# nvpro-samples/vk_raytrace

Measured on AMD Instinct MI355X. Metric: Msamples/s on Sponza 1920x1080; per-pixel L2 vs ref at equal spp, higher is better.
Workload: dtype f32; 1 GPU; C3 sponza-like (synthetic Crytek-Sponza stand-in, 262267 tris target) 1920x1080 589spp depth8 Disney + HDR env; triangles=269004, materials=23, textures=43, width=1920, height=1080, spp=589, max_depth=8, bsdf=disney, env=2048x1024 procedural HDR, parallelism=image tiles 32x32 over 1 GPU(s), scene replicated

## Files before the change

include/pt_fpmath.h:

```cpp
#ifndef PT_FPMATH_H
#define PT_FPMATH_H

#include <math.h>
#include <stdint.h>
#include <string.h>

#if defined(__HIPCC__)
#define PT_FP __host__ __device__ __forceinline__
#else
#define PT_FP static inline
#endif

PT_FP float ptf_from_bits(uint32_t u)
{
  float f;
  memcpy(&f, &u, 4);
  return f;
}
PT_FP uint32_t ptf_bits(float f)
{
  uint32_t u;
  memcpy(&u, &f, 4);
  return u;
}
// ... 49 lines not shown
  if(ptf_abs(x) < 2.44140625e-4f)
    return x;
  float r;
  int   q;
  ptf_sincos_reduce(x, &r, &q);
  float v = (q & 1) ? ptf_cos_kernel(r) : ptf_sin_kernel(r);
  return (q & 2) ? -v : v;
}
PT_FP float pt_cos(float x)
{
  float r;
  int   q;
  ptf_sincos_reduce(x, &r, &q);
  float v = (q & 1) ? ptf_sin_kernel(r) : ptf_cos_kernel(r);
  return ((q + 1) & 2) ? -v : v;
}
PT_FP float pt_tan(float x)
{
  if(ptf_abs(x) < 2.44140625e-4f)
    return x;
  float r;
  int   q;
  ptf_sincos_reduce(x, &r, &q);
  float s = ptf_sin_kernel(r), c = ptf_cos_kernel(r);
  return (q & 1) ? -c / s : s / c;
}

PT_FP float ptf_asin_poly(float x, float z)
{
  float p = ptf_fma(3.3921066672e-02f, z, 1.7005795613e-02f);
// ... 262 lines not shown
```

include/pt_types.h:

```cpp
#ifndef PT_TYPES_H
#define PT_TYPES_H

#include <stdint.h>

#ifdef __cplusplus
extern "C" {
#endif

#define PT_TILE 32

enum pt_DebugMode {
  PT_DEBUG_NONE = 0,
  PT_DEBUG_BASECOLOR = 1,
  PT_DEBUG_NORMAL = 2,
  PT_DEBUG_METALLIC = 3,
  PT_DEBUG_EMISSIVE = 4,
  PT_DEBUG_ALPHA = 5,
  PT_DEBUG_ROUGHNESS = 6,
  PT_DEBUG_TEXCOORD = 7,
  PT_DEBUG_TANGENT = 8,
  PT_DEBUG_RADIANCE = 9,
  PT_DEBUG_WEIGHT = 10,
  PT_DEBUG_RAYDIR = 11,
  PT_DEBUG_HEATMAP = 12
// ... 121 lines not shown
typedef struct pt_PrimMesh {
  uint32_t vertexOffset;
  uint32_t vertexCount;
  uint32_t firstIndex;
  uint32_t indexCount;
  int32_t  materialIndex;
} pt_PrimMesh;

typedef struct pt_Node {
  float   worldMatrix[16];
  int32_t primMesh;
} pt_Node;

enum { PT_VARIANT_RAYQUERY = 0, PT_VARIANT_RTX = 1 };
enum { PT_ACCEL_FLAT = 0, PT_ACCEL_TWO_LEVEL = 1 };
enum { PT_FN_SIN = 0, PT_FN_COS, PT_FN_TAN, PT_FN_ASIN, PT_FN_ACOS, PT_FN_ATAN2, PT_FN_EXP, PT_FN_LOG, PT_FN_POW };
enum { PT_FILTER_NEAREST = 0, PT_FILTER_LINEAR = 1 };
enum { PT_WRAP_REPEAT = 0, PT_WRAP_MIRRORED_REPEAT = 1, PT_WRAP_CLAMP_TO_EDGE = 2 };

typedef struct pt_TextureDesc {
  const uint8_t* rgba8;
  int32_t        width;
  int32_t        height;
  int32_t        magFilter;
  int32_t        minFilter;
  int32_t        wrapS;
  int32_t        wrapT;
} pt_TextureDesc;

typedef struct pt_SceneDesc {
  const pt_VertexAttributes*  vertices;
// ... 108 lines not shown
```

vk_raytrace_amd/capi.py:

```python
import ctypes as C
import os

import numpy as np

from . import host_device as hd

PT_VARIANT_RAYQUERY, PT_VARIANT_RTX = 0, 1
PT_ACCEL_FLAT, PT_ACCEL_TWO_LEVEL = 0, 1
PT_RAYS_CLOSEST, PT_RAYS_OCCLUDED, PT_RAYS_NEAREST, PT_RAYS_CANDIDATES = 0, 1, 2, 3
PT_RAY_HIT, PT_RAY_INVALID = 1, 2
PT_RAYS_DEVICE = 1
PT_RAYS_MAX_HITS = 16
PT_QUERY_CHUNK = 1 << 20
PT_DISPLAY_RING = 8
PT_FN = {"sin": 0, "cos": 1, "tan": 2, "asin": 3, "acos": 4, "atan2": 5, "exp": 6, "log": 7, "pow": 8}
PT_OK, PT_ERR_INVALID, PT_ERR_NO_DEVICE, PT_ERR_HIP, PT_ERR_STATE, PT_ERR_OOM, PT_ERR_UNAVAILABLE = 0, -1, -2, -3, -4, -5, -6

LIB_PATH = os.environ.get("PT_LIB") or os.path.join(os.path.dirname(os.path.abspath(__file__)), "libptmi.so")

_P = C.c_void_p
API = [
    ("pt_create", C.c_int, [C.c_int, C.POINTER(_P)]),
    ("pt_destroy", C.c_int, [_P]),
    ("pt_renderer_name", C.c_char_p, []),
    ("pt_last_error", C.c_char_p, [_P]),
    ("pt_set_scene", C.c_int, [_P, C.POINTER(hd.SceneDesc)]),
    ("pt_build_accel", C.c_int, [_P]),
    ("pt_set_accel_mode", C.c_int, [_P, C.c_int]),
    ("pt_update_instances", C.c_int, [_P, _P, C.c_uint32]),
    ("pt_set_camera", C.c_int, [_P, C.POINTER(hd.SceneCamera)]),
# ... 128 lines not shown
```

vk_raytrace_amd/csrc/pt_bsdf.h:

```cpp
#pragma once
#include "pt_surface.h"

PT_DEV float schlick_weight(float u)
{
  float m  = clampf(1.0f - u, 0.0f, 1.0f);
  float m2 = m * m;
  return m2 * m2 * m;
}
PT_DEV float fresnel_dielectric(float cosI, float eta)
{
  float sinT2 = eta * eta * (1.0f - cosI * cosI);
  if(sinT2 > 1.0f)
    return 1.0f;
  float cosT = sqrtf(fmax2(1.0f - sinT2, 0.0f));
  float rs   = (eta * cosT - cosI) / (eta * cosT + cosI);
  float rp   = (eta * cosI - cosT) / (eta * cosI + cosT);
  return 0.5f * (rs * rs + rp * rp);
}
PT_DEV float gtr1(float NdotH, float a)
{
  if(a >= 1.0f)
    return PT_1_OVER_PI;
  float a2 = a * a;
  float t  = 1.0f + (a2 - 1.0f) * NdotH * NdotH;
// ... 13 lines not shown
  return 1.0f / (PT_PI * ax * ay * c * c);
}
PT_DEV float smith_ggx(float NdotV, float alphaG)
{
  float a = alphaG * alphaG;
  float b = NdotV * NdotV;
  return 1.0f / (NdotV + sqrtf(a + b - a * b));
}
PT_DEV float smith_ggx_aniso(float NdotV, float VdotX, float VdotY, float ax, float ay)
{
  float a = VdotX * ax;
  float b = VdotY * ay;
  float c = NdotV;
  return 1.0f / (NdotV + sqrtf(a * a + b * b + c * c));
}
PT_DEV f3 sample_cosine_hemisphere(float r1, float r2)
{
  float r   = sqrtf(r1);
  float phi = PT_TWO_PI * r2;
  f3    d;
  d.x = r * pt_cos(phi);
  d.y = r * pt_sin(phi);
  d.z = sqrtf(fmax2(0.0f, 1.0f - d.x * d.x - d.y * d.y));
  return d;
}
PT_DEV f3 sample_uniform_hemisphere(float r1, float r2)
{
  float r   = sqrtf(fmax2(0.0f, 1.0f - r1 * r1));
  float phi = PT_TWO_PI * r2;
  return f3{r * pt_cos(phi), r * pt_sin(phi), r1};
}
PT_DEV float power_heuristic(float a, float b)
{
  float t = a * a;
  return t / (b * b + t);
}
PT_DEV f3 sample_gtr1(float rgh, float r1)
{
  float a        = fmax2(0.001f, rgh);
  float a2       = a * a;
  float phi      = r1 * PT_TWO_PI;
  float cosTheta = sqrtf((1.0f - pt_pow(a2, 1.0f - r1)) / (1.0f - a2));
  float sinTheta = clampf(sqrtf(1.0f - (cosTheta * cosTheta)), 0.0f, 1.0f);
  return f3{sinTheta * pt_cos(phi), sinTheta * pt_sin(phi), cosTheta};
}
PT_DEV f3 sample_gtr2_aniso(float ax, float ay, float r1, float r2)
{
  float phi      = r1 * PT_TWO_PI;
  float sinPhi   = ay * pt_sin(phi);
  float cosPhi   = ax * pt_cos(phi);
  float tanTheta = sqrtf(r2 / (1 - r2));
  return f3{tanTheta * cosPhi, tanTheta * sinPhi, 1.0f};
}
PT_DEV f3 sample_gtr2(float rgh, float r1, float r2)
{
  float a        = fmax2(0.001f, rgh);
  float phi      = r1 * PT_TWO_PI;
  float cosTheta = sqrtf((1.0f - r2) / (1.0f + (a * a - 1.0f) * r2));
  float sinTheta = clampf(sqrtf(1.0f - (cosTheta * cosTheta)), 0.0f, 1.0f);
  return f3{sinTheta * pt_cos(phi), sinTheta * pt_sin(phi), cosTheta};
}

PT_DEV f3 disney_reflection(const Surface& s, float eta, f3 V, f3 N, f3 L, f3 H, float& pdf)
{
  if(dot3(N, L) < 0.0f)
    return splat3(0.0f);
  float F = fresnel_dielectric(dot3(V, H), eta);
  float D = gtr2(dot3(N, H), s.roughness);
  pdf     = D * dot3(N, H) * F / (4.0f * dot3(V, H));
  float G = smith_ggx(fabsf(dot3(N, L)), s.roughness) * smith_ggx(dot3(N, V), s.roughness);
  return s.albedo * F * D * G;
}
PT_DEV f3 disney_refraction(const Surface& s, float eta, f3 V, f3 N, f3 L, f3 H, float& pdf)
{
  float F     = fresnel_dielectric(fabsf(dot3(V, H)), eta);
// ... 43 lines not shown
{
  pdf      = (1.0f / PT_TWO_PI);
  float FL = schlick_weight(fabsf(dot3(N, L)));
  float FV = schlick_weight(dot3(N, V));
  float Fd = (1.0f - 0.5f * FL) * (1.0f - 0.5f * FV);
  return sqrt3(s.albedo) * s.subsurface * (1.0f / PT_PI) * Fd * (1.0f - s.metallic) * (1.0f - s.transmission);
}
PT_DEV f3 disney_spec_tint(const Surface& s)
{
  f3    Cdlin = s.albedo;
  float Cdlum = 0.3f * Cdlin.x + 0.6f * Cdlin.y + 0.1f * Cdlin.z;
  f3    Ctint = Cdlum > 0.0f ? Cdlin / Cdlum : splat3(1.0f);
  return lerp(lerp(splat3(1.0f), Ctint, s.specularTint) * (s.specular * 0.08f), Cdlin, s.metallic);
}

PT_DEV f3 disney_sample(const Surface& s, f3 V, f3 N, f3& L, float& pdf, uint32_t& seed)
{
  pdf  = 0.0f;
  f3 f = splat3(0.0f);

  float r1 = rng_next(seed);
  float r2 = rng_next(seed);

  float diffuseRatio = 0.5f * (1.0f - s.metallic);
  float transWeight  = (1.0f - s.metallic) * s.transmission;
  f3    Cspec0       = disney_spec_tint(s);
  f3    Csheen       = s.sheenTint;

  if(rng_next(seed) < transWeight)
  {
    f3 H = sample_gtr2(s.roughness, r1, r2);
    H    = s.tangent * H.x + s.bitangent * H.y + N * H.z;

    f3    R   = mirror(-V, H);
    float eta = s.eta;
    float F   = fresnel_dielectric(fabsf(dot3(R, H)), eta);
    if(s.thinwalled)
    {
      if(dot3(s.ffnormal, s.normal) < 0.0f)
        F = 0;
      eta = 1.001f;
    }
    if(rng_next(seed) < F)
    {
      L = unit(R);
      f = disney_reflection(s, eta, V, N, L, H, pdf);
    }
    else
    {
      L = unit(bend(-V, H, eta));
      f = disney_refraction(s, eta, V, N, L, H, pdf);
    }
    f *= transWeight;
    pdf *= transWeight;
  }
  else
  {
    if(rng_next(seed) < diffuseRatio)
    {
      if(rng_next(seed) < s.subsurface)
      {
        L = sample_uniform_hemisphere(r1, r2);
        L = s.tangent * L.x + s.bitangent * L.y - N * L.z;
        f = disney_subsurface(s, V, N, L, pdf);
        pdf *= s.subsurface * diffuseRatio;
      }
      else
      {
        L    = sample_cosine_hemisphere(r1, r2);
        L    = s.tangent * L.x + s.bitangent * L.y + N * L.z;
        f3 H = unit(L + V);
        f    = disney_diffuse(s, Csheen, V, N, L, H, pdf);
        pdf *= (1.0f - s.subsurface) * diffuseRatio;
      }
    }
    else
    {
      float primarySpecRatio = 1.0f / (1.0f + s.clearcoat);
      if(rng_next(seed) < primarySpecRatio)
      {
        f3 H = sample_gtr2_aniso(s.ax, s.ay, r1, r2);
        H    = s.tangent * H.x + s.bitangent * H.y + N * H.z;
        L    = unit(mirror(-V, H));
        f    = disney_specular(s, Cspec0, V, N, L, H, pdf);
        pdf *= primarySpecRatio * (1.0f - diffuseRatio);
      }
      else
      {
        f3 H = sample_gtr1(s.clearcoatRoughness, r1);
        H    = s.tangent * H.x + s.bitangent * H.y + N * H.z;
        L    = unit(mirror(-V, H));
        f    = disney_clearcoat(s, V, N, L, H, pdf);
        pdf *= (1.0f - primarySpecRatio) * (1.0f - diffuseRatio);
      }
    }
    f *= (1.0f - transWeight);
    pdf *= (1.0f - transWeight);
  }
  return f;
}

PT_DEV f3 disney_eval(const Surface& s, f3 V, f3 N, f3 L, float& pdf)
{
  f3 H;
  if(dot3(N, L) < 0.0f)
    H = unit(L * (1.0f / s.eta) + V);
  else
    H = unit(L + V);
  if(dot3(N, H) < 0.0f)
// ... 59 lines not shown
  return clampf(v, 0.0f, 1.0f);
}
PT_DEV float gltf_d_ggx(float NdotH, float alphaRoughness)
{
  float a2 = alphaRoughness * alphaRoughness;
  float f  = (NdotH * NdotH) * (a2 - 1.0f) + 1.0f;
  return a2 / (PT_PI * f * f);
}
PT_DEV float gltf_d_ggx_aniso(float NdotH, float TdotH, float BdotH, float at, float ab)
{
  float a2 = at * ab;
  f3    f  = f3{ab * TdotH, at * BdotH, a2 * NdotH};
  float w2 = a2 / dot3(f, f);
  return a2 * w2 * w2 / PT_PI;
}
PT_DEV f3 gltf_ggx_halfvector(float alpha, float r1, float r2)
{
  float phi      = r1 * 2.0f * PT_PI;
  float cosTheta = sqrtf((1.0f - r2) / (1.0f + (alpha * alpha - 1.0f) * r2));
  float sinTheta = clampf(sqrtf(1.0f - (cosTheta * cosTheta)), 0.0f, 1.0f);
  return f3{sinTheta * pt_cos(phi), sinTheta * pt_sin(phi), cosTheta};
}
PT_DEV f3 gltf_diffuse(const Surface& s, f3 V, f3 N, f3 L, float& pdf)
{
  pdf         = 0;
  float NdotV = dot3(N, V);
  float NdotL = dot3(N, L);
  if(NdotL < 0.0f || NdotV < 0.0f)
    return splat3(0.0f);
  NdotL = clampf(NdotL, 0.001f, 1.0f);
  pdf   = NdotL * PT_1_OVER_PI;
  return (s.albedo / PT_PI) * (1.0f - s.metallic);
}
PT_DEV f3 gltf_specular(const Surface& s, f3 f0, f3 f90, f3 V, f3 N, f3 L, f3 H, float& pdf)
{
  pdf         = 0;
// ... 91 lines not shown
  return lerp(brdf, bsdf, transWeight);
}

PT_DEV f3 gltf_sample(const Surface& s, f3 V, f3 N, f3& L, float& pdf, uint32_t& seed)
{
  pdf     = 0.0f;
  f3 brdf = splat3(0.0f);

  float probability   = rng_next(seed);
  float diffuseRatio  = 0.5f * (1.0f - s.metallic);
  float specularRatio = 1.0f - diffuseRatio;
  float transWeight   = (1.0f - s.metallic) * s.transmission;
  float r1            = rng_next(seed);
  float r2            = rng_next(seed);

  if(rng_next(seed) < transWeight)
  {
    float eta   = s.eta;
    float n2    = s.ior;
    float R0    = (1.0f - n2) / (1.0f + n2);
    f3    H     = gltf_ggx_halfvector(s.roughness, r1, r2);
    H           = s.tangent * H.x + s.bitangent * H.y + N * H.z;
    float VdotH = dot3(V, H);
    float F     = gltf_fresnel(R0 * R0, 1.0f, VdotH);
    float disc  = 1.0f - eta * eta * (1.0f - VdotH * VdotH);
    if(s.thinwalled)
    {
      if(dot3(s.ffnormal, s.normal) < 0.0f)
      {
        F    = 0;
        disc = 0;
      }
      eta = 1.00f;
    }
    if(disc < 0.0f || rng_next(seed) < F)
    {
// ... 3 lines not shown
    {
      L = unit(bend(-V, H, eta));
      if(isnan(L.x) || isnan(L.y) || isnan(L.z))
        L = -V;
    }
    pdf  = fabsf(dot3(N, L));
    brdf = s.albedo;
  }
  else
  {
    f3 f0, f90;
    gltf_f0_f90(s, f0, f90);
    f3 T = s.tangent, B = s.bitangent;
    if(probability < diffuseRatio)
    {
      L    = sample_cosine_hemisphere(r1, r2);
      L    = T * L.x + B * L.y + N * L.z;
      brdf = gltf_diffuse(s, V, N, L, pdf);
      pdf *= (1.0f - s.subsurface) * diffuseRatio;
    }
    else
    {
      float primarySpecRatio = 1.0f / (1.0f + s.clearcoat);
      float roughness        = (rng_next(seed) < primarySpecRatio) ? s.roughness : s.clearcoatRoughness;
      f3    H                = gltf_ggx_halfvector(roughness, r1, r2);
      H                      = T * H.x + B * H.y + N * H.z;
      L                      = mirror(-V, H);
      if(rng_next(seed) < primarySpecRatio)
      {
        brdf = gltf_specular(s, f0, f90, V, N, L, H, pdf);
        pdf *= primarySpecRatio * specularRatio;
      }
      else
      {
        brdf = gltf_clearcoat(s, V, N, L, H, pdf);
        pdf *= (1.0f - primarySpecRatio) * specularRatio;
      }
    }
    brdf *= (1.0f - transWeight);
    pdf *= (1.0f - transWeight);
// ... 4 lines not shown
```

vk_raytrace_amd/csrc/pt_capi.hip:

```cpp
#include <algorithm>
#include <atomic>
#include <cstdlib>
#include <cstring>
#include "pt_context.h"
#include "pt_scene_records.h"

static std::string g_createError;

int dev_alloc(pt_context* c, DevBuf& b, size_t bytes)
{
  if(b.p && b.bytes >= bytes && b.bytes <= bytes * 2 + 4096)
    return PT_OK;
  dev_free(b);
  if(bytes == 0)
    bytes = 16;
  HIP_TRY(c, hipMalloc(&b.p, bytes));
  b.bytes = bytes;
  return PT_OK;
}
bool dev_alloc_quiet(DevBuf& b, size_t bytes)
{
  if(b.p && b.bytes >= bytes && b.bytes <= bytes * 2 + 4096)
    return true;
  dev_free(b);
// ... 427 lines not shown
}

int pt_set_env(pt_context* c, const float* rgba, int w, int h, float* out_integral, float* out_average)
{
  CTX_CHECK(c);
  if(!rgba || w <= 0 || h <= 0)
    return c->fail(PT_ERR_INVALID, "pt_set_env: bad image");
  HIP_TRY(c, hipSetDevice(c->device));
  HIP_TRY(c, sync_all(c));
  std::vector<pt_EnvAccel> accel(size_t(w) * h);
  float                    integral = 1.f, average = 1.f;
  if(pt_build_env_accel(rgba, w, h, accel.data(), &integral, &average) != PT_OK)
    return c->fail(PT_ERR_INVALID, "pt_build_env_accel failed");
  int rc;
  if((rc = upload(c, c->dEnv, rgba, sizeof(float) * 4 * size_t(w) * h)) != PT_OK) return rc;
  if((rc = upload(c, c->dEnvAccel, accel.data(), sizeof(pt_EnvAccel) * accel.size())) != PT_OK) return rc;
  c->scene.envW = w;
  c->scene.envH = h;
  c->haveEnv    = true;
  refresh_scene_ptrs(c);
  if(out_integral) *out_integral = integral;
  if(out_average) *out_average = average;
  return PT_OK;
}

int pt_set_variant(pt_context* c, int variant)
{
  CTX_CHECK(c);
  if(variant != PT_VARIANT_RAYQUERY && variant != PT_VARIANT_RTX)
    return c->fail(PT_ERR_INVALID, "pt_set_variant: %d", variant);
  int rc = flush_pending(c);
// ... 766 lines not shown
```

vk_raytrace_amd/csrc/pt_debug.hip:

```cpp
#include <algorithm>
#include "pt_context.h"
#include "pt_probe.h"

extern "C" {

__global__ void __launch_bounds__(256) k_calib_valu(int iters, float* out)
{
  float a0 = threadIdx.x, a1 = a0 + 1.f, a2 = a0 + 2.f, a3 = a0 + 3.f, a4 = a0 + 4.f, a5 = a0 + 5.f, a6 = a0 + 6.f, a7 = a0 + 7.f;
  const float m = 0.999f, c = 0.001f;
  for(int i = 0; i < iters; ++i)
  {
    asm volatile("v_fmac_f32 %0, %8, %9\n v_fmac_f32 %1, %8, %9\n v_fmac_f32 %2, %8, %9\n v_fmac_f32 %3, %8, %9\n"
                 "v_fmac_f32 %4, %8, %9\n v_fmac_f32 %5, %8, %9\n v_fmac_f32 %6, %8, %9\n v_fmac_f32 %7, %8, %9\n"
                 : "+v"(a0), "+v"(a1), "+v"(a2), "+v"(a3), "+v"(a4), "+v"(a5), "+v"(a6), "+v"(a7)
                 : "v"(m), "v"(c));
  }
  float s = ((a0 + a1) + (a2 + a3)) + ((a4 + a5) + (a6 + a7));
  if(s == 12345.678f)
    out[0] = s;
}
__global__ void __launch_bounds__(256) k_calib_copy(const float4* __restrict__ src, float4* __restrict__ dst, size_t n)
{
  for(size_t i = size_t(blockIdx.x) * blockDim.x + threadIdx.x; i < n; i += size_t(gridDim.x) * blockDim.x)
    dst[i] = src[i];
// ... 63 lines not shown
{
  uint64_t i = uint64_t(blockIdx.x) * blockDim.x + threadIdx.x;
  if(i >= n)
    return;
  float x = a[i], y = b ? b[i] : 0.0f, r;
  switch(fn)
  {
    case PT_FN_SIN: r = pt_sin(x); break;
    case PT_FN_COS: r = pt_cos(x); break;
    case PT_FN_TAN: r = pt_tan(x); break;
    case PT_FN_ASIN: r = pt_asin(x); break;
    case PT_FN_ACOS: r = pt_acos(x); break;
    case PT_FN_ATAN2: r = pt_atan2(x, y); break;
    case PT_FN_EXP: r = pt_exp(x); break;
    case PT_FN_LOG: r = pt_log(x); break;
    default: r = pt_pow(x, y); break;
  }
  out[i] = r;
}
int pt_fpmath_eval(pt_context* c, int fn, uint64_t n, const float* a, const float* b, float* out)
{
  CTX_CHECK(c);
  if(fn < PT_FN_SIN || fn > PT_FN_POW || !a || !out || ((fn == PT_FN_ATAN2 || fn == PT_FN_POW) && !b))
    return c->fail(PT_ERR_INVALID, "pt_fpmath_eval: bad arguments");
  if(n == 0)
    return PT_OK;
  HIP_TRY(c, hipSetDevice(c->device));
  float *dA = nullptr, *dB = nullptr, *dO = nullptr;
  int    rc = PT_OK;
  auto   done = [&](int r) {
    (void)hipFree(dA); (void)hipFree(dB); (void)hipFree(dO);
    return r;
  };
  if(hipMalloc(&dA, n * 4) != hipSuccess || hipMalloc(&dO, n * 4) != hipSuccess || (b && hipMalloc(&dB, n * 4) != hipSuccess))
    return done(c->fail(PT_ERR_OOM, "pt_fpmath_eval: out of device memory"));
  if(hipMemcpy(dA, a, n * 4, hipMemcpyHostToDevice) != hipSuccess || (b && hipMemcpy(dB, b, n * 4, hipMemcpyHostToDevice) != hipSuccess))
    return done(c->fail(PT_ERR_HIP, "pt_fpmath_eval: upload failed"));
  k_fpmath<<<dim3((unsigned)((n + 255) / 256)), dim3(256), 0, c->stream>>>(fn, n, dA, dB, dO);
  if(hipStreamSynchronize(c->stream) != hipSuccess || hipMemcpy(out, dO, n * 4, hipMemcpyDeviceToHost) != hipSuccess)
    return done(c->fail(PT_ERR_HIP, "pt_fpmath_eval: kernel failed"));
  return done(rc);
}

}

template <class Launch>
static int run_rows(pt_context* c, const char* who, uint32_t n, const float* in, int in_stride, float* out, int out_stride, Launch&& launch)
{
  float *dIn = nullptr, *dOut = nullptr;
  auto   done = [&](int r) {
    (void)hipFree(dIn); (void)hipFree(dOut);
    return r;
  };
  const size_t inBytes = size_t(n) * in_stride * 4, outBytes = size_t(n) * out_stride * 4;
// ... 170 lines not shown
```

vk_raytrace_amd/csrc/pt_device.h:

```cpp
#pragma once
#include "../../include/pt_types.h"
#include "pt_math.h"
#include <cstring>

struct TriRec {
  float4 p0w;
  float4 e1n;
  float4 e2p;
};
#define TRI_OPAQUE 1u
#define TRI_NOCULL 2u
#define TRI_FLIP 4u
#define TRI_INDEX_MASK 0x1fffffffu

struct BvhNode {
  float4 a;
  float4 b;
  float4 c;
  uint4  d;
};
#define BVH_LEAF 0x80000000u
#define BVH_ALPHA 0x40000000u
#define BVH_SLOT_MASK 0x3fffffffu
#define BVH_NONE 0xffffffffu
// ... 138 lines not shown
         eq(m.attenuationColor[2], one) && eq(m.thicknessFactor, zero) && eq(m.attenuationDistance, big) && eq(m.clearcoatFactor, zero) &&
         eq(m.clearcoatRoughness, zero) && m.clearcoatTexture == -1 && m.clearcoatRoughnessTexture == -1 && m.sheen == 0u;
}
inline void mat_line_pack(const pt_GltfShadeMaterial& m, const TexRec rec[4], uint4 out[PT_MAT_LINE_QUADS])
{
  auto bits = [](float f) { uint32_t u; std::memcpy(&u, &f, 4); return u; };
  const int      ids[4] = {m.normalTexture, m.emissiveTexture, m.pbrMetallicRoughnessTexture, m.pbrBaseColorTexture};
  const uint32_t flags  = (ids[0] > -1 ? MAT_HAS_NORMAL : 0u) | (ids[1] > -1 ? MAT_HAS_EMISSIVE : 0u) | (ids[2] > -1 ? MAT_HAS_MR : 0u) | (ids[3] > -1 ? MAT_HAS_BASE : 0u) |
                         (mat_is_simple(m) ? MAT_SIMPLE : 0u);
  out[0] = uint4{bits(m.pbrBaseColorFactor[0]), bits(m.pbrBaseColorFactor[1]), bits(m.pbrBaseColorFactor[2]), bits(m.pbrBaseColorFactor[3])};
  out[1] = uint4{bits(m.emissiveFactor[0]), bits(m.emissiveFactor[1]), bits(m.emissiveFactor[2]), bits(m.normalTextureScale)};
  out[2] = uint4{bits(m.pbrRoughnessFactor), bits(m.pbrMetallicFactor), bits(m.ior), flags};
  for(int k = 0; k < 4; ++k)
    out[3 + k] = tex_desc_pack(rec[k]);
  out[7] = uint4{0u, 0u, 0u, 0u};
}

#define PT_SHADE_REC_QUADS 8
struct DeviceScene {
  const float4*               vertices;
  const uint32_t*             indices;
  const InstanceRec*          instances;
  const pt_GltfShadeMaterial* materials;
  const pt_Light*             lights;
  const TexRec*               texRecs;
  const uint4*                matLines;
  const uint32_t*             texels;
  const BvhNode*              bvh;
  const WideNode*             wide;
  const CompactNode*          cnodes;
  const float4*               shadeTris;
  const TriRec*               tris;
  const AlphaRec*             alphaRecs;
  const AlphaMat*             alphaMats;
  const uint32_t*             alphaMaps;
  const float4*               env;
  const pt_EnvAccel*          envAccel;
  int32_t                     envW, envH;
  uint32_t                    numTris;
  uint32_t                    numInstances;
  pt_SceneCamera              camera;
  pt_SunAndSky                sunsky;
  float                       boundsMin[3];
  float                       boundsInvExt[3];
  const WideNode*             tlas;
  const CompactNode*          ctlas;
  const TlasLeaf*             tlasLeaves;
  const uint32_t*             instTriBase;
  const uint32_t*             instBlock;
  uint32_t                    twoLevel;
  uint32_t                    allOpaque;
};

#define PT_STATE_PLAIN 0
#define PT_STATE_NT 1
#ifndef PT_STATE_POLICY
#define PT_STATE_POLICY PT_STATE_NT
#endif
template <int POL>
struct StateArrayT {
  float4* p;
  PT_DEV float4& operator[](size_t i) const { return p[i]; }
  PT_DEV operator float4*() const { return p; }
};
#if defined(__HIP_DEVICE_COMPILE__)
typedef float pt_nt_f4 __attribute__((ext_vector_type(4)));
struct StateF1RefNt {
// ... 63 lines not shown
```

vk_raytrace_amd/csrc/pt_probe.h:

```cpp
#pragma once
#include "pt_shade.h"
#include "pt_cnode.h"

enum {
  PROBE_EVAL_DISNEY = 0, PROBE_EVAL_GLTF, PROBE_SAMPLE_DISNEY, PROBE_SAMPLE_GLTF, PROBE_SUN_AND_SKY, PROBE_SPHERICAL_UV, PROBE_FRAME, PROBE_RANGE_ATTENUATION,
  PROBE_SPOT_ATTENUATION, PROBE_MIRROR, PROBE_BEND, PROBE_LERP, PROBE_SMOOTH, PROBE_ENV_SAMPLE, PROBE_CROSS, PROBE_UNIT, PROBE_MAT4_VEC4, PROBE_VEC4_MAT4,
  PROBE_XFORM_POINT, PROBE_XFORM_ROWVEC, PROBE_XFORM_DIR, PROBE_BASIS_MUL, PROBE_COUNT
};
enum { PROBE_BSDF_IN = 40, PROBE_ENV_TEXELS = 8, PROBE_SKY_WORDS = int(sizeof(pt_SunAndSky) / 4) };

__host__ __device__ inline void probe_row_words(int fn, int& in, int& out)
{
  switch(fn)
  {
    case PROBE_EVAL_DISNEY: case PROBE_EVAL_GLTF: in = PROBE_BSDF_IN; out = 4; break;
    case PROBE_SAMPLE_DISNEY: case PROBE_SAMPLE_GLTF: in = PROBE_BSDF_IN; out = 8; break;
    case PROBE_SUN_AND_SKY: in = PROBE_SKY_WORDS + 3; out = 3; break;
    case PROBE_SPHERICAL_UV: in = 3; out = 2; break;
    case PROBE_FRAME: in = 3; out = 6; break;
    case PROBE_RANGE_ATTENUATION: in = 2; out = 1; break;
    case PROBE_SPOT_ATTENUATION: in = 8; out = 1; break;
    case PROBE_MIRROR: in = 6; out = 3; break;
    case PROBE_BEND: case PROBE_LERP: in = 7; out = 3; break;
    case PROBE_SMOOTH: in = 3; out = 1; break;
    case PROBE_ENV_SAMPLE: in = 8 + 4 * PROBE_ENV_TEXELS; out = 4; break;
    case PROBE_CROSS: in = 6; out = 3; break;
    case PROBE_UNIT: in = 3; out = 3; break;
    case PROBE_MAT4_VEC4: in = 20; out = 4; break;
    case PROBE_XFORM_POINT: case PROBE_XFORM_ROWVEC: case PROBE_XFORM_DIR: in = 15; out = 3; break;
    case PROBE_BASIS_MUL: in = 12; out = 3; break;
    default: in = 0; out = 0; break;
  }
}

PT_DEV f3 probe_f3(const float* p) { return f3{p[0], p[1], p[2]}; }
PT_DEV void probe_put(float* o, f3 v) { o[0] = v.x; o[1] = v.y; o[2] = v.z; }

PT_DEV void probe_surface(Surface& s, const float* r)
{
  const float* m = r;
// ... 53 lines not shown
    case PROBE_FRAME:
    {
      f3 T, B;
      make_frame(probe_f3(in), T, B);
      probe_put(out, T);
      probe_put(out + 3, B);
      break;
    }
    case PROBE_RANGE_ATTENUATION: out[0] = range_attenuation(in[0], in[1]); break;
    case PROBE_SPOT_ATTENUATION: out[0] = spot_attenuation(probe_f3(in), probe_f3(in + 3), in[6], in[7]); break;
    case PROBE_MIRROR: probe_put(out, mirror(probe_f3(in), probe_f3(in + 3))); break;
    case PROBE_BEND: probe_put(out, bend(probe_f3(in), probe_f3(in + 3), in[6])); break;
    case PROBE_LERP: probe_put(out, lerp(probe_f3(in), probe_f3(in + 3), in[6])); break;
    case PROBE_SMOOTH: out[0] = smooth(in[0], in[1], in[2]); break;
    case PROBE_ENV_SAMPLE:
    {
      const int w = int(in[3]), h = int(in[4]);
      if(w < 1 || h < 1 || w * h > PROBE_ENV_TEXELS)
        break;
      pt_EnvAccel acc[PROBE_ENV_TEXELS];
      float4      texels[PROBE_ENV_TEXELS];
      for(int k = 0; k < PROBE_ENV_TEXELS; ++k)
      {
        acc[k].alias = __float_as_uint(in[8 + 4 * k]); acc[k].q = in[9 + 4 * k]; acc[k].pdf = in[10 + 4 * k]; acc[k].aliasPdf = in[11 + 4 * k];
        texels[k] = make_float4(1.0f, 1.0f, 1.0f, 1.0f);
      }
      DeviceScene S;
      memset(&S, 0, sizeof(S));
      S.env = texels; S.envAccel = acc; S.envW = w; S.envH = h;
      f3    toLight = splat3(0.0f);
      float pdf     = 0.0f;
      (void)env_importance_sample(S, probe_f3(in), toLight, pdf);
      probe_put(out, toLight);
      out[3] = pdf;
      break;
    }
    case PROBE_CROSS: probe_put(out, cross3(probe_f3(in), probe_f3(in + 3))); break;
    case PROBE_UNIT: probe_put(out, unit(probe_f3(in))); break;
    case PROBE_MAT4_VEC4:
    {
      const f4 r = mat4_mul(in, f4{in[16], in[17], in[18], in[19]});
      out[0] = r.x; out[1] = r.y; out[2] = r.z; out[3] = r.w;
      break;
    }
// ... 341 lines not shown
```

vk_raytrace_amd/csrc/pt_shade.h:

```cpp
#pragma once
#include "pt_bsdf.h"
#include "pt_internal.h"
#include "pt_sky.h"
#include "pt_settle.h"

enum { SHADE_DONE = 0, SHADE_TO_SHADOW = 1, SHADE_TO_NEXT = 2 };
enum { EV_MISS = 1u, EV_HIT = 2u, EV_NEE = 4u };

PT_DEV bool slot_pixel(const FrameParams& fp, const uint32_t* slotTile, uint32_t slot, int& px, int& py)
{
  uint32_t gt = slotTile[slot >> 10];
  uint32_t in = slot & 1023u, blk = in >> 6, lane = in & 63u;
  px          = int(gt % uint32_t(fp.tilesX)) * PT_TILE + int(blk & 3u) * 8 + int(lane & 7u);
  py          = int(gt / uint32_t(fp.tilesX)) * PT_TILE + int(blk >> 2) * 8 + int(lane >> 3);
  return px < fp.width && py < fp.height;
}

PT_DEV f4 mat4_mul(const float* m, f4 v)
{
  f4 c0 = f4{m[0], m[1], m[2], m[3]}, c1 = f4{m[4], m[5], m[6], m[7]}, c2 = f4{m[8], m[9], m[10], m[11]}, c3 = f4{m[12], m[13], m[14], m[15]};
  return ((c0 * v.x + c1 * v.y) + c2 * v.z) + c3 * v.w;
}

PT_DEV f2 spherical_uv(f3 v)
// ... 41 lines not shown
  f2 center = f2{float(px), float(py)} + jitter;
  f2 inUV   = f2{center.x / float(st.size[0]), center.y / float(st.size[1])};
  f2 d      = inUV * 2.0f - f2{1.0f, 1.0f};

  const pt_SceneCamera& cam = S.camera;
  f4 origin    = mat4_mul(cam.viewInverse, f4{0, 0, 0, 1});
  f4 target    = mat4_mul(cam.projInverse, f4{d.x, d.y, 1, 1});
  f3 tn        = unit(xyz(target));
  f4 direction = mat4_mul(cam.viewInverse, f4{tn.x, tn.y, tn.z, 0});

  f3    focalPoint = xyz(direction) * cam.focalDist;
  float cam_r1     = rng_next(seed) * PT_TWO_PI;
  float cam_r2     = rng_next(seed) * cam.aperture;
  f4    cam_right  = mat4_mul(cam.viewInverse, f4{1, 0, 0, 0});
  f4    cam_up     = mat4_mul(cam.viewInverse, f4{0, 1, 0, 0});
  f3    lens       = (xyz(cam_right) * pt_cos(cam_r1) + xyz(cam_up) * pt_sin(cam_r1)) * sqrtf(cam_r2);
  dir              = unit(focalPoint - lens);
  org              = xyz(origin) + lens;
}
PT_DEV void generate_ray(const DeviceScene& S, const RenderBuffers& rb, const FrameParams& fp, uint32_t slot, uint32_t fb, int px, int py)
{
  uint32_t seed = fp.sample == 0 ? 0u : __float_as_uint(rb.ps.rayD[slot].w);
  f3       org, dir;
  camera_ray(S, fp, fb, px, py, seed, org, dir);
  rb.ps.rayO[slot]   = make_float4(org.x, org.y, org.z, 0.f);
  rb.ps.rayD[slot]   = make_float4(dir.x, dir.y, dir.z, __uint_as_float(seed));
  if(fp.st.maxDepth == 0)
    rb.ps.rad[slot] = make_float4(0.f, 0.f, 0.f, 0.f);
}

PT_DEV f3 env_importance_sample(const DeviceScene& S, f3 xi, f3& toLight, float& pdf)
// ... 5 lines not shown
  const pt_EnvAccel e    = S.envAccel[idx];
  uint32_t          envIdx;
  if(xi.y < e.q)
  {
    envIdx = idx;
    xi.y /= e.q;
    pdf = e.pdf;
  }
  else
  {
    envIdx = e.alias;
    xi.y   = (xi.y - e.q) / (1.0f - e.q);
    pdf    = e.aliasPdf;
  }
  const uint32_t px = envIdx % width, py = envIdx / width;
  const float    u        = (float(px) + xi.y) / float(width);
  const float    phi      = u * (2.0f * PT_PI) - PT_PI;
  const float    sin_phi  = pt_sin(phi), cos_phi = pt_cos(phi);
  const float    step     = PT_PI / float(height);
  const float    theta0   = float(py) * step;
  const float    cosTheta = pt_cos(theta0) * (1.0f - xi.z) + pt_cos(theta0 + step) * xi.z;
  const float    theta    = pt_acos(cosTheta);
  const float    sinTheta = pt_sin(theta);
  const float    v        = theta * PT_1_OVER_PI;
  toLight                 = f3{cos_phi * sinTheta, cosTheta, sin_phi * sinTheta};
  return sample_env(S, f2{u, v});
}

PT_DEV float range_attenuation(float range, float distance)
{
  if(range <= 0.0f)
    return 1.0f;
  return fmax2(fmin2(1.0f - pt_pow(distance / range, 4.0f), 1.0f), 0.0f) / pt_pow(distance, 2.0f);
}
PT_DEV float spot_attenuation(f3 pointToLight, f3 spotDir, float outerCos, float innerCos)
{
// ... 114 lines not shown
    }
    rb.ps.rad[slot] = make_float4(r.x, r.y, r.z, 0.f);
    return SHADE_DONE;
  }
  if(sf.unlit)
  {
    f3 r            = radiance + sf.albedo * throughput;
    rb.ps.rad[slot] = make_float4(r.x, r.y, r.z, 0.f);
    return SHADE_DONE;
  }

  f3 absorption = depth == 0 ? splat3(0.0f) : xyz(rb.ps.absorb[slot]);
  if(dot3(sf.normal, sf.ffnormal) > 0.0f)
    absorption = splat3(0.0f);
  radiance += sf.emission * throughput;
  throughput *= exp3(-absorption * hit.x);

  f3    neeRadiance = splat3(0.0f), lightDir = splat3(0.0f);
  float lightDist = 1e32f;
  bool  visible   = false;
  {
    f3    lightContrib;
    float lightPdf;
    bool  isLight = false;
    float pSelect = st.hdrMultiplier > 0.0f ? 0.5f : 1.0f;
    if(nbLights != 0 && rng_next(seed) <= pSelect)
    {
      isLight            = true;
      int            li  = int(fmin2(rng_next(seed) * float(nbLights), float(nbLights)));
      li                 = li < nbLights - 1 ? li : nbLights - 1;
      const pt_Light lt  = S.lights[li];
// ... 173 lines not shown
```

Before: 1635 Msamples/s.

## Fuse sin/cos into sincos, tabulate env row cosines, skip trivial absorption exp

Adds a fused pt_sincos that shares one range reduction between sine and cosine. It is used in BSDF sampling (the lobe is now picked up front so phi is computed once), in the camera lens sampling and in env importance sampling. Env row boundary cosines are precomputed on the host and appended to the envAccel buffer, which replaces two cos calls per env sample with one table load. The absorption exp3 is skipped when absorption is zero. The trade-offs are branch restructuring in disney_sample, an extra scattered memory read per env sample, and possible tiny numerical differences.

Result: no change. 1631 Msamples/s (-0.3%).

```diff
diff --git a/include/pt_fpmath.h b/include/pt_fpmath.h
--- a/include/pt_fpmath.h
+++ b/include/pt_fpmath.h
@@ -87,6 +87,18 @@
   ptf_sincos_reduce(x, &r, &q);
   float v = (q & 1) ? ptf_sin_kernel(r) : ptf_cos_kernel(r);
   return ((q + 1) & 2) ? -v : v;
+}
+PT_FP void pt_sincos(float x, float* s, float* c)
+{
+  float r;
+  int   q;
+  ptf_sincos_reduce(x, &r, &q);
+  float sk = ptf_sin_kernel(r), ck = ptf_cos_kernel(r);
+  float sv = (q & 1) ? ck : sk;
+  float cv = (q & 1) ? sk : ck;
+  sv       = (q & 2) ? -sv : sv;
+  *c       = ((q + 1) & 2) ? -cv : cv;
+  *s       = (ptf_abs(x) < 2.44140625e-4f) ? x : sv;
 }
 PT_FP float pt_tan(float x)
 {
diff --git a/include/pt_types.h b/include/pt_types.h
--- a/include/pt_types.h
+++ b/include/pt_types.h
@@ -159,7 +159,7 @@
 
 enum { PT_VARIANT_RAYQUERY = 0, PT_VARIANT_RTX = 1 };
 enum { PT_ACCEL_FLAT = 0, PT_ACCEL_TWO_LEVEL = 1 };
-enum { PT_FN_SIN = 0, PT_FN_COS, PT_FN_TAN, PT_FN_ASIN, PT_FN_ACOS, PT_FN_ATAN2, PT_FN_EXP, PT_FN_LOG, PT_FN_POW };
+enum { PT_FN_SIN = 0, PT_FN_COS, PT_FN_TAN, PT_FN_ASIN, PT_FN_ACOS, PT_FN_ATAN2, PT_FN_EXP, PT_FN_LOG, PT_FN_POW, PT_FN_SINCOS  };
 enum { PT_FILTER_NEAREST = 0, PT_FILTER_LINEAR = 1 };
 enum { PT_WRAP_REPEAT = 0, PT_WRAP_MIRRORED_REPEAT = 1, PT_WRAP_CLAMP_TO_EDGE = 2 };
 
diff --git a/vk_raytrace_amd/capi.py b/vk_raytrace_amd/capi.py
--- a/vk_raytrace_amd/capi.py
+++ b/vk_raytrace_amd/capi.py
@@ -13,7 +13,7 @@
 PT_RAYS_MAX_HITS = 16
 PT_QUERY_CHUNK = 1 << 20
 PT_DISPLAY_RING = 8
-PT_FN = {"sin": 0, "cos": 1, "tan": 2, "asin": 3, "acos": 4, "atan2": 5, "exp": 6, "log": 7, "pow": 8}
+PT_FN = {"sin": 0, "cos": 1, "tan": 2, "asin": 3, "acos": 4, "atan2": 5, "exp": 6, "log": 7, "pow": 8, "sincos": 9}
 PT_OK, PT_ERR_INVALID, PT_ERR_NO_DEVICE, PT_ERR_HIP, PT_ERR_STATE, PT_ERR_OOM, PT_ERR_UNAVAILABLE = 0, -1, -2, -3, -4, -5, -6
 
 LIB_PATH = os.environ.get("PT_LIB") or os.path.join(os.path.dirname(os.path.abspath(__file__)), "libptmi.so")
diff --git a/vk_raytrace_amd/csrc/pt_bsdf.h b/vk_raytrace_amd/csrc/pt_bsdf.h
--- a/vk_raytrace_amd/csrc/pt_bsdf.h
+++ b/vk_raytrace_amd/csrc/pt_bsdf.h
@@ -51,51 +51,46 @@
   float c = NdotV;
   return 1.0f / (NdotV + sqrtf(a * a + b * b + c * c));
 }
-PT_DEV f3 sample_cosine_hemisphere(float r1, float r2)
-{
-  float r   = sqrtf(r1);
-  float phi = PT_TWO_PI * r2;
+PT_DEV f3 sample_cosine_hemisphere(float r1, float sinPhi, float cosPhi)
+{
+  float r = sqrtf(r1);
   f3    d;
-  d.x = r * pt_cos(phi);
-  d.y = r * pt_sin(phi);
+  d.x = r * cosPhi;
+  d.y = r * sinPhi;
   d.z = sqrtf(fmax2(0.0f, 1.0f - d.x * d.x - d.y * d.y));
   return d;
 }
-PT_DEV f3 sample_uniform_hemisphere(float r1, float r2)
-{
-  float r   = sqrtf(fmax2(0.0f, 1.0f - r1 * r1));
-  float phi = PT_TWO_PI * r2;
-  return f3{r * pt_cos(phi), r * pt_sin(phi), r1};
+PT_DEV f3 sample_uniform_hemisphere(float r1, float sinPhi, float cosPhi)
+{
+  float r = sqrtf(fmax2(0.0f, 1.0f - r1 * r1));
+  return f3{r * cosPhi, r * sinPhi, r1};
 }
 PT_DEV float power_heuristic(float a, float b)
 {
   float t = a * a;
   return t / (b * b + t);
 }
-PT_DEV f3 sample_gtr1(float rgh, float r1)
+PT_DEV f3 sample_gtr1(float rgh, float r1, float sinPhi, float cosPhi)
 {
   float a        = fmax2(0.001f, rgh);
   float a2       = a * a;
-  float phi      = r1 * PT_TWO_PI;
   float cosTheta = sqrtf((1.0f - pt_pow(a2, 1.0f - r1)) / (1.0f - a2));
   float sinTheta = clampf(sqrtf(1.0f - (cosTheta * cosTheta)), 0.0f, 1.0f);
-  return f3{sinTheta * pt_cos(phi), sinTheta * pt_sin(phi), cosTheta};
-}
-PT_DEV f3 sample_gtr2_aniso(float ax, float ay, float r1, float r2)
-{
-  float phi      = r1 * PT_TWO_PI;
-  float sinPhi   = ay * pt_sin(phi);
-  float cosPhi   = ax * pt_cos(phi);
+  return f3{sinTheta * cosPhi, sinTheta * sinPhi, cosTheta};
+}
+PT_DEV f3 sample_gtr2_aniso(float ax, float ay, float r2, float sinPhi, float cosPhi)
+{
+  float sinP     = ay * sinPhi;
+  float cosP     = ax * cosPhi;
   float tanTheta = sqrtf(r2 / (1 - r2));
-  return f3{tanTheta * cosPhi, tanTheta * sinPhi, 1.0f};
-}
-PT_DEV f3 sample_gtr2(float rgh, float r1, float r2)
+  return f3{tanTheta * cosP, tanTheta * sinP, 1.0f};
+}
+PT_DEV f3 sample_gtr2(float rgh, float r2, float sinPhi, float cosPhi)
 {
   float a        = fmax2(0.001f, rgh);
-  float phi      = r1 * PT_TWO_PI;
   float cosTheta = sqrtf((1.0f - r2) / (1.0f + (a * a - 1.0f) * r2));
   float sinTheta = clampf(sqrtf(1.0f - (cosTheta * cosTheta)), 0.0f, 1.0f);
-  return f3{sinTheta * pt_cos(phi), sinTheta * pt_sin(phi), cosTheta};
+  return f3{sinTheta * cosPhi, sinTheta * sinPhi, cosTheta};
 }
 
 PT_DEV f3 disney_reflection(const Surface& s, float eta, f3 V, f3 N, f3 L, f3 H, float& pdf)
@@ -169,6 +164,8 @@
   return lerp(lerp(splat3(1.0f), Ctint, s.specularTint) * (s.specular * 0.08f), Cdlin, s.metallic);
 }
 
+enum { LOBE_TRANSMISSION = 0, LOBE_SUBSURFACE, LOBE_DIFFUSE, LOBE_SPECULAR, LOBE_CLEARCOAT };
+
 PT_DEV f3 disney_sample(const Surface& s, f3 V, f3 N, f3& L, float& pdf, uint32_t& seed)
 {
   pdf  = 0.0f;
@@ -182,9 +179,24 @@
   f3    Cspec0       = disney_spec_tint(s);
   f3    Csheen       = s.sheenTint;
 
-  if(rng_next(seed) < transWeight)
-  {
-    f3 H = sample_gtr2(s.roughness, r1, r2);
+  int   lobe             = LOBE_TRANSMISSION;
+  float primarySpecRatio = 0.0f;
+  if(!(rng_next(seed) < transWeight))
+  {
+    if(rng_next(seed) < diffuseRatio)
+      lobe = rng_next(seed) < s.subsurface ? LOBE_SUBSURFACE : LOBE_DIFFUSE;
+    else
+    {
+      primarySpecRatio = 1.0f / (1.0f + s.clearcoat);
+      lobe             = rng_next(seed) < primarySpecRatio ? LOBE_SPECULAR : LOBE_CLEARCOAT;
+    }
+  }
+  float sinPhi, cosPhi;
+  pt_sincos(((lobe == LOBE_SUBSURFACE || lobe == LOBE_DIFFUSE) ? r2 : r1) * PT_TWO_PI, &sinPhi, &cosPhi);
+
+  if(lobe == LOBE_TRANSMISSION)
+  {
+    f3 H = sample_gtr2(s.roughness, r2, sinPhi, cosPhi);
     H    = s.tangent * H.x + s.bitangent * H.y + N * H.z;
 
     f3    R   = mirror(-V, H);
@@ -211,43 +223,36 @@
   }
   else
   {
-    if(rng_next(seed) < diffuseRatio)
-    {
-      if(rng_next(seed) < s.subsurface)
-      {
-        L = sample_uniform_hemisphere(r1, r2);
-        L = s.tangent * L.x + s.bitangent * L.y - N * L.z;
-        f = disney_subsurface(s, V, N, L, pdf);
-        pdf *= s.subsurface * diffuseRatio;
-      }
-      else
-      {
-        L    = sample_cosine_hemisphere(r1, r2);
-        L    = s.tangent * L.x + s.bitangent * L.y + N * L.z;
-        f3 H = unit(L + V);
-        f    = disney_diffuse(s, Csheen, V, N, L, H, pdf);
-        pdf *= (1.0f - s.subsurface) * diffuseRatio;
-      }
-    }
-    else
-    {
-      float primarySpecRatio = 1.0f / (1.0f + s.clearcoat);
-      if(rng_next(seed) < primarySpecRatio)
-      {
-        f3 H = sample_gtr2_aniso(s.ax, s.ay, r1, r2);
-        H    = s.tangent * H.x + s.bitangent * H.y + N * H.z;
-        L    = unit(mirror(-V, H));
-        f    = disney_specular(s, Cspec0, V, N, L, H, pdf);
-        pdf *= primarySpecRatio * (1.0f - diffuseRatio);
-      }
-      else
-      {
-        f3 H = sample_gtr1(s.clearcoatRoughness, r1);
-        H    = s.tangent * H.x + s.bitangent * H.y + N * H.z;
-        L    = unit(mirror(-V, H));
-        f    = disney_clearcoat(s, V, N, L, H, pdf);
-        pdf *= (1.0f - primarySpecRatio) * (1.0f - diffuseRatio);
-      }
+    if(lobe == LOBE_SUBSURFACE)
+    {
+      L = sample_uniform_hemisphere(r1, sinPhi, cosPhi);
+      L = s.tangent * L.x + s.bitangent * L.y - N * L.z;
+      f = disney_subsurface(s, V, N, L, pdf);
+      pdf *= s.subsurface * diffuseRatio;
+    }
+    else if(lobe == LOBE_DIFFUSE)
+    {
+      L    = sample_cosine_hemisphere(r1, sinPhi, cosPhi);
+      L    = s.tangent * L.x + s.bitangent * L.y + N * L.z;
+      f3 H = unit(L + V);
+      f    = disney_diffuse(s, Csheen, V, N, L, H, pdf);
+      pdf *= (1.0f - s.subsurface) * diffuseRatio;
+    }
+    else if(lobe == LOBE_SPECULAR)
+    {
+      f3 H = sample_gtr2_aniso(s.ax, s.ay, r2, sinPhi, cosPhi);
+      H    = s.tangent * H.x + s.bitangent * H.y + N * H.z;
+      L    = unit(mirror(-V, H));
+      f    = disney_specular(s, Cspec0, V, N, L, H, pdf);
+      pdf *= primarySpecRatio * (1.0f - diffuseRatio);
+    }
+    else
+    {
+      f3 H = sample_gtr1(s.clearcoatRoughness, r1, sinPhi, cosPhi);
+      H    = s.tangent * H.x + s.bitangent * H.y + N * H.z;
+      L    = unit(mirror(-V, H));
+      f    = disney_clearcoat(s, V, N, L, H, pdf);
+      pdf *= (1.0f - primarySpecRatio) * (1.0f - diffuseRatio);
     }
     f *= (1.0f - transWeight);
     pdf *= (1.0f - transWeight);
@@ -337,12 +342,11 @@
   float w2 = a2 / dot3(f, f);
   return a2 * w2 * w2 / PT_PI;
 }
-PT_DEV f3 gltf_ggx_halfvector(float alpha, float r1, float r2)
-{
-  float phi      = r1 * 2.0f * PT_PI;
+PT_DEV f3 gltf_ggx_halfvector(float alpha, float r2, float sinPhi, float cosPhi)
+{
   float cosTheta = sqrtf((1.0f - r2) / (1.0f + (alpha * alpha - 1.0f) * r2));
   float sinTheta = clampf(sqrtf(1.0f - (cosTheta * cosTheta)), 0.0f, 1.0f);
-  return f3{sinTheta * pt_cos(phi), sinTheta * pt_sin(phi), cosTheta};
+  return f3{sinTheta * cosPhi, sinTheta * sinPhi, cosTheta};
 }
 PT_DEV f3 gltf_diffuse(const Surface& s, f3 V, f3 N, f3 L, float& pdf)
 {
@@ -464,12 +468,16 @@
   float r1            = rng_next(seed);
   float r2            = rng_next(seed);
 
-  if(rng_next(seed) < transWeight)
+  const bool trans = rng_next(seed) < transWeight;
+  float      sinPhi, cosPhi;
+  pt_sincos(((!trans && probability < diffuseRatio) ? r2 : r1) * 2.0f * PT_PI, &sinPhi, &cosPhi);
+
+  if(trans)
   {
     float eta   = s.eta;
     float n2    = s.ior;
     float R0    = (1.0f - n2) / (1.0f + n2);
-    f3    H     = gltf_ggx_halfvector(s.roughness, r1, r2);
+    f3    H     = gltf_ggx_halfvector(s.roughness, r2, sinPhi, cosPhi);
     H           = s.tangent * H.x + s.bitangent * H.y + N * H.z;
     float VdotH = dot3(V, H);
     float F     = gltf_fresnel(R0 * R0, 1.0f, VdotH);
@@ -503,7 +511,7 @@
     f3 T = s.tangent, B = s.bitangent;
     if(probability < diffuseRatio)
     {
-      L    = sample_cosine_hemisphere(r1, r2);
+      L    = sample_cosine_hemisphere(r1, sinPhi, cosPhi);
       L    = T * L.x + B * L.y + N * L.z;
       brdf = gltf_diffuse(s, V, N, L, pdf);
       pdf *= (1.0f - s.subsurface) * diffuseRatio;
@@ -512,7 +520,7 @@
     {
       float primarySpecRatio = 1.0f / (1.0f + s.clearcoat);
       float roughness        = (rng_next(seed) < primarySpecRatio) ? s.roughness : s.clearcoatRoughness;
-      f3    H                = gltf_ggx_halfvector(roughness, r1, r2);
+      f3    H                = gltf_ggx_halfvector(roughness, r2, sinPhi, cosPhi);
       H                      = T * H.x + B * H.y + N * H.z;
       L                      = mirror(-V, H);
       if(rng_next(seed) < primarySpecRatio)
diff --git a/vk_raytrace_amd/csrc/pt_capi.hip b/vk_raytrace_amd/csrc/pt_capi.hip
--- a/vk_raytrace_amd/csrc/pt_capi.hip
+++ b/vk_raytrace_amd/csrc/pt_capi.hip
@@ -465,7 +465,13 @@
     return c->fail(PT_ERR_INVALID, "pt_build_env_accel failed");
   int rc;
   if((rc = upload(c, c->dEnv, rgba, sizeof(float) * 4 * size_t(w) * h)) != PT_OK) return rc;
-  if((rc = upload(c, c->dEnvAccel, accel.data(), sizeof(pt_EnvAccel) * accel.size())) != PT_OK) return rc;
+  std::vector<unsigned char> blob(sizeof(pt_EnvAccel) * accel.size() + sizeof(float2) * size_t(h));
+  std::memcpy(blob.data(), accel.data(), sizeof(pt_EnvAccel) * accel.size());
+  float2* rowCos = reinterpret_cast<float2*>(blob.data() + sizeof(pt_EnvAccel) * accel.size());
+  for(int py = 0; py < h; ++py)
+    rowCos[py] = env_row_cos(uint32_t(py), uint32_t(h));
+  if((rc = upload(c, c->dEnvAccel, blob.data(), blob.size())) != PT_OK) return rc;
+  c->scene.envRowTable = 1u;
   c->scene.envW = w;
   c->scene.envH = h;
   c->haveEnv    = true;
diff --git a/vk_raytrace_amd/csrc/pt_debug.hip b/vk_raytrace_amd/csrc/pt_debug.hip
--- a/vk_raytrace_amd/csrc/pt_debug.hip
+++ b/vk_raytrace_amd/csrc/pt_debug.hip
@@ -101,6 +101,7 @@
     case PT_FN_ATAN2: r = pt_atan2(x, y); break;
     case PT_FN_EXP: r = pt_exp(x); break;
     case PT_FN_LOG: r = pt_log(x); break;
+    case PT_FN_SINCOS: pt_sincos(x, &r, &out[n + i]); break;
     default: r = pt_pow(x, y); break;
   }
   out[i] = r;
@@ -108,7 +109,7 @@
 int pt_fpmath_eval(pt_context* c, int fn, uint64_t n, const float* a, const float* b, float* out)
 {
   CTX_CHECK(c);
-  if(fn < PT_FN_SIN || fn > PT_FN_POW || !a || !out || ((fn == PT_FN_ATAN2 || fn == PT_FN_POW) && !b))
+  if(fn < PT_FN_SIN || fn > PT_FN_SINCOS || !a || !out || ((fn == PT_FN_ATAN2 || fn == PT_FN_POW) && !b))
     return c->fail(PT_ERR_INVALID, "pt_fpmath_eval: bad arguments");
   if(n == 0)
     return PT_OK;
@@ -119,12 +120,13 @@
     (void)hipFree(dA); (void)hipFree(dB); (void)hipFree(dO);
     return r;
   };
-  if(hipMalloc(&dA, n * 4) != hipSuccess || hipMalloc(&dO, n * 4) != hipSuccess || (b && hipMalloc(&dB, n * 4) != hipSuccess))
+  const size_t outBytes = n * 4 * (fn == PT_FN_SINCOS ? 2 : 1);
+  if(hipMalloc(&dA, n * 4) != hipSuccess || hipMalloc(&dO, outBytes) != hipSuccess || (b && hipMalloc(&dB, n * 4) != hipSuccess))
     return done(c->fail(PT_ERR_OOM, "pt_fpmath_eval: out of device memory"));
   if(hipMemcpy(dA, a, n * 4, hipMemcpyHostToDevice) != hipSuccess || (b && hipMemcpy(dB, b, n * 4, hipMemcpyHostToDevice) != hipSuccess))
     return done(c->fail(PT_ERR_HIP, "pt_fpmath_eval: upload failed"));
   k_fpmath<<<dim3((unsigned)((n + 255) / 256)), dim3(256), 0, c->stream>>>(fn, n, dA, dB, dO);
-  if(hipStreamSynchronize(c->stream) != hipSuccess || hipMemcpy(out, dO, n * 4, hipMemcpyDeviceToHost) != hipSuccess)
+  if(hipStreamSynchronize(c->stream) != hipSuccess || hipMemcpy(out, dO, outBytes, hipMemcpyDeviceToHost) != hipSuccess)
     return done(c->fail(PT_ERR_HIP, "pt_fpmath_eval: kernel failed"));
   return done(rc);
 }
diff --git a/vk_raytrace_amd/csrc/pt_device.h b/vk_raytrace_amd/csrc/pt_device.h
--- a/vk_raytrace_amd/csrc/pt_device.h
+++ b/vk_raytrace_amd/csrc/pt_device.h
@@ -176,6 +176,16 @@
   for(int k = 0; k < 4; ++k)
     out[3 + k] = tex_desc_pack(rec[k]);
   out[7] = uint4{0u, 0u, 0u, 0u};
+}
+
+#if defined(__HIPCC__)
+__host__ __device__
+#endif
+inline float2 env_row_cos(uint32_t py, uint32_t height)
+{
+  const float step   = PT_PI / float(height);
+  const float theta0 = float(py) * step;
+  return make_float2(pt_cos(theta0), pt_cos(theta0 + step));
 }
 
 #define PT_SHADE_REC_QUADS 8
@@ -205,6 +215,7 @@
   pt_SunAndSky                sunsky;
   float                       boundsMin[3];
   float                       boundsInvExt[3];
+  uint32_t                    envRowTable;
   const WideNode*             tlas;
   const CompactNode*          ctlas;
   const TlasLeaf*             tlasLeaves;
@@ -213,6 +224,13 @@
   uint32_t                    twoLevel;
   uint32_t                    allOpaque;
 };
+#if defined(__HIPCC__)
+__host__ __device__
+#endif
+inline const float2* env_row_table(const DeviceScene& S)
+{
+  return S.envRowTable ? reinterpret_cast<const float2*>(S.envAccel + size_t(uint32_t(S.envW) * uint32_t(S.envH))) : nullptr;
+}
 
 #define PT_STATE_PLAIN 0
 #define PT_STATE_NT 1
diff --git a/vk_raytrace_amd/csrc/pt_probe.h b/vk_raytrace_amd/csrc/pt_probe.h
--- a/vk_raytrace_amd/csrc/pt_probe.h
+++ b/vk_raytrace_amd/csrc/pt_probe.h
@@ -5,7 +5,7 @@
 enum {
   PROBE_EVAL_DISNEY = 0, PROBE_EVAL_GLTF, PROBE_SAMPLE_DISNEY, PROBE_SAMPLE_GLTF, PROBE_SUN_AND_SKY, PROBE_SPHERICAL_UV, PROBE_FRAME, PROBE_RANGE_ATTENUATION,
   PROBE_SPOT_ATTENUATION, PROBE_MIRROR, PROBE_BEND, PROBE_LERP, PROBE_SMOOTH, PROBE_ENV_SAMPLE, PROBE_CROSS, PROBE_UNIT, PROBE_MAT4_VEC4, PROBE_VEC4_MAT4,
-  PROBE_XFORM_POINT, PROBE_XFORM_ROWVEC, PROBE_XFORM_DIR, PROBE_BASIS_MUL, PROBE_COUNT
+  PROBE_XFORM_POINT, PROBE_XFORM_ROWVEC, PROBE_XFORM_DIR, PROBE_BASIS_MUL, PROBE_SUN_DISK, PROBE_ENV_SAMPLE_TABLE, PROBE_COUNT
 };
 enum { PROBE_BSDF_IN = 40, PROBE_ENV_TEXELS = 8, PROBE_SKY_WORDS = int(sizeof(pt_SunAndSky) / 4) };
 
@@ -23,7 +23,7 @@
     case PROBE_MIRROR: in = 6; out = 3; break;
     case PROBE_BEND: case PROBE_LERP: in = 7; out = 3; break;
     case PROBE_SMOOTH: in = 3; out = 1; break;
-    case PROBE_ENV_SAMPLE: in = 8 + 4 * PROBE_ENV_TEXELS; out = 4; break;
+    case PROBE_ENV_SAMPLE: case PROBE_ENV_SAMPLE_TABLE: in = 8 + 4 * PROBE_ENV_TEXELS; out = 4; break;
     case PROBE_CROSS: in = 6; out = 3; break;
     case PROBE_UNIT: in = 3; out = 3; break;
     case PROBE_MAT4_VEC4: in = 20; out = 4; break;
@@ -107,11 +107,12 @@
     case PROBE_LERP: probe_put(out, lerp(probe_f3(in), probe_f3(in + 3), in[6])); break;
     case PROBE_SMOOTH: out[0] = smooth(in[0], in[1], in[2]); break;
     case PROBE_ENV_SAMPLE:
+    case PROBE_ENV_SAMPLE_TABLE:
     {
       const int w = int(in[3]), h = int(in[4]);
       if(w < 1 || h < 1 || w * h > PROBE_ENV_TEXELS)
         break;
-      pt_EnvAccel acc[PROBE_ENV_TEXELS];
+      pt_EnvAccel acc[PROBE_ENV_TEXELS + PROBE_ENV_TEXELS / 2];
       float4      texels[PROBE_ENV_TEXELS];
       for(int k = 0; k < PROBE_ENV_TEXELS; ++k)
       {
@@ -121,6 +122,13 @@
       DeviceScene S;
       memset(&S, 0, sizeof(S));
       S.env = texels; S.envAccel = acc; S.envW = w; S.envH = h;
+      if(fn == PROBE_ENV_SAMPLE_TABLE)
+      {
+        float2* rowCos = reinterpret_cast<float2*>(acc + w * h);
+        for(int py = 0; py < h; ++py)
+          rowCos[py] = env_row_cos(uint32_t(py), uint32_t(h));
+        S.envRowTable = 1u;
+      }
       f3    toLight = splat3(0.0f);
       float pdf     = 0.0f;
       (void)env_importance_sample(S, probe_f3(in), toLight, pdf);
diff --git a/vk_raytrace_amd/csrc/pt_shade.h b/vk_raytrace_amd/csrc/pt_shade.h
--- a/vk_raytrace_amd/csrc/pt_shade.h
+++ b/vk_raytrace_amd/csrc/pt_shade.h
@@ -79,7 +79,9 @@
   float cam_r2     = rng_next(seed) * cam.aperture;
   f4    cam_right  = mat4_mul(cam.viewInverse, f4{1, 0, 0, 0});
   f4    cam_up     = mat4_mul(cam.viewInverse, f4{0, 1, 0, 0});
-  f3    lens       = (xyz(cam_right) * pt_cos(cam_r1) + xyz(cam_up) * pt_sin(cam_r1)) * sqrtf(cam_r2);
+  float cam_sin, cam_cos;
+  pt_sincos(cam_r1, &cam_sin, &cam_cos);
+  f3    lens       = (xyz(cam_right) * cam_cos + xyz(cam_up) * cam_sin) * sqrtf(cam_r2);
   dir              = unit(focalPoint - lens);
   org              = xyz(origin) + lens;
 }
@@ -115,12 +117,13 @@
     pdf    = e.aliasPdf;
   }
   const uint32_t px = envIdx % width, py = envIdx / width;
+  const float2*  rowTable = env_row_table(S);
+  const float2   rowCos   = rowTable ? rowTable[py] : env_row_cos(py, height);
   const float    u        = (float(px) + xi.y) / float(width);
   const float    phi      = u * (2.0f * PT_PI) - PT_PI;
-  const float    sin_phi  = pt_sin(phi), cos_phi = pt_cos(phi);
-  const float    step     = PT_PI / float(height);
-  const float    theta0   = float(py) * step;
-  const float    cosTheta = pt_cos(theta0) * (1.0f - xi.z) + pt_cos(theta0 + step) * xi.z;
+  float          sin_phi, cos_phi;
+  pt_sincos(phi, &sin_phi, &cos_phi);
+  const float    cosTheta = rowCos.x * (1.0f - xi.z) + rowCos.y * xi.z;
   const float    theta    = pt_acos(cosTheta);
   const float    sinTheta = pt_sin(theta);
   const float    v        = theta * PT_1_OVER_PI;
@@ -265,7 +268,8 @@
   if(dot3(sf.normal, sf.ffnormal) > 0.0f)
     absorption = splat3(0.0f);
   radiance += sf.emission * throughput;
-  throughput *= exp3(-absorption * hit.x);
+  if(!(absorption.x == 0.0f && absorption.y == 0.0f && absorption.z == 0.0f && fabsf(hit.x) <= 3.4028234e38f))
+    throughput *= exp3(-absorption * hit.x);
 
   f3    neeRadiance = splat3(0.0f), lightDir = splat3(0.0f);
   float lightDist = 1e32f;
```
